# penumbra-zone/decaf377

Hardware: AMD Instinct MI355X
Metric: decaf377 var-base scalar-mults/sec + encodes/sec at 1/2/4/8 MI355X (higher is better)
Workload: dtype u32

## Files before the change

### decaf377_amd/csrc/batch_host.hpp

```cpp
#pragma once
#include <hip/hip_runtime.h>
#include <stdint.h>
#include <stdio.h>
#include <stdlib.h>

#include "dcb.hpp"
#include "straus.hpp"
#include "host_state.hpp"

namespace d377 {

inline int lane_residency(const void* fn, const char* name, int bits, int& lds) {
  if (lds >= 0) return D377_OK;
  int nb = 0;
  HIP_TRY(hipOccupancyMaxActiveBlocksPerMultiprocessor(&nb, fn, BLOCK, 0));
  int pad = 0;
  if (nb > WAVES_PER_SIMD) {
    pad = (160 * 1024) / (WAVES_PER_SIMD + 1) + 1024;
    if (pad > 64 * 1024) HIP_TRY(hipFuncSetAttribute(fn, hipFuncAttributeMaxDynamicSharedMemorySize, pad));
    HIP_TRY(hipOccupancyMaxActiveBlocksPerMultiprocessor(&nb, fn, BLOCK, (size_t)pad));
  }
  if (getenv("D377_DEBUG_RESIDENCY"))
    fprintf(stderr, "d377: %s<%d>: %d workgroups per CU with %d bytes of LDS padding\n", name, bits, nb, pad);
  if (nb < 1 || nb > WAVES_PER_SIMD)
    return fail(D377_ERR_INIT, "residency of %s does not match the lane sets of the scratch areas", name);
  lds = pad;
  return D377_OK;
}

inline int straus_scratch_reserve(DeviceState& d, hipStream_t s, size_t terms, const char* in_capture, const char* no_memory,
                                  uint32_t** tab, uint32_t** dig) {
  const size_t tab_words = d.resident_lanes() * terms * VB_ENTRIES * BM_ENTRY_WORDS;
  const size_t need = (tab_words + d.resident_lanes() * BM_WINDOWS) * sizeof(uint32_t);
  if (need > d.bm_cap) {
    if (ScratchGuard::capturing(s)) return fail(D377_ERR_ARG, "%s", in_capture);
    int rc;
    if ((rc = d.vb_guard.drain())) return rc;
    if (d.bm_scratch) HIP_TRY(hipFree(d.bm_scratch));
    d.bm_scratch = nullptr; d.bm_cap = 0;
    if (hipMalloc(&d.bm_scratch, need) != hipSuccess) {
      (void)hipGetLastError();
      return fail(D377_ERR_HIP, "%s", no_memory);
    }
    d.bm_cap = need;
  }
  *tab = d.bm_scratch;
  *dig = d.bm_scratch + tab_words;
  return D377_OK;
}

inline DcbScratch lane_chunks(const DeviceState& d, size_t count, int* grid, int kmax = DCB_K) {
  const size_t places = (size_t)d.cus * WAVES_PER_SIMD;
  const ChunkDeal c = deal_chunks((count + BLOCK - 1) / BLOCK, places, (size_t)kmax, (size_t)d.cus * 64);
  DcbScratch dcb{d.dcb_scratch, d.slot_pool, d.cus * WAVES_PER_SIMD, (int)c.per_lane, d.dcb_sets * BLOCK, (int)c.extra, d.pool_health};
  dcb.prio = c.nchunks <= 2 * places ? 1 : 0;
  *grid = (int)c.nchunks;
  return dcb;
}

template <class Body>
int device_slice(DeviceState& d, Body&& body) {
  HIP_TRY(hipSetDevice(d.id));
  int rc = D377_OK;
  SyncOnError guard{&rc, d.id, d.stream, nullptr};
  rc = [&]() -> int {
    StarveCheck starve{d, d.stream};
    int r;
    if ((r = starve.before())) return r;
    if ((r = body())) return r;
    if ((r = starve.after())) return r;
    HIP_TRY(hipStreamSynchronize(d.stream));
    return starve.verdict();
  }();
  return rc;
}

inline int sums_out_reserve(DeviceState& d, size_t n, bool want_xyzt, uint64_t** xyzt_dev) {
  int rc;
  if ((rc = ensure(d, 2, n * (want_xyzt ? 32 + 128 : 32)))) return rc;
  *xyzt_dev = want_xyzt ? reinterpret_cast<uint64_t*>(d.buf[2] + n * 32) : nullptr;
  return D377_OK;
}
inline int sums_out_copy(DeviceState& d, size_t n, uint8_t* out32, uint64_t* xyzt_out) {
  HIP_TRY(hipMemcpyAsync(out32, d.buf[2], n * 32, hipMemcpyDeviceToHost, d.stream));
  if (xyzt_out) HIP_TRY(hipMemcpyAsync(xyzt_out, d.buf[2] + n * 32, n * 128, hipMemcpyDeviceToHost, d.stream));
// ... 5 lines not shown
```

### decaf377_amd/csrc/batch_msm.hip

```cpp
#include <hip/hip_runtime.h>
#include <stdint.h>
#include <stdlib.h>
#include <string.h>

#include "../../include/decaf377_amd.h"
#include "curve.hpp"
#include "device_util.hpp"
#include "dcb.hpp"
#include "quad_ops.hpp"
#include "row_ops.hpp"
#include "straus.hpp"
#include "straus_tab.hpp"
#include "host_state.hpp"
#include "batch_host.hpp"

using namespace d377;

namespace {

constexpr int BM_MAX = D377_BATCH_MSM_MAX_TERMS;
static_assert(BM_MAX == 8, "a window's digits of the m points of a sum are the eight nibbles of one word");
static_assert(VB_ENTRIES == 9, "straus_sum stores entries 0 .. 8 of every point's table");

template <bool ENCODED>
__global__ void __launch_bounds__(BLOCK, WAVES_PER_SIMD)
k_batch_msm_lane(SqrtTables T, const void* pts_in, const uint8_t* scalar32, int m, size_t n, uint8_t* out32, uint64_t* xyzt_out,
                 uint8_t* status, uint32_t* tab, uint32_t* dig, DcbScratch dcb) {
  __shared__ uint32_t lds_pow_[ENCODED ? POW_TAB * NL * BLOCK : 1];
  LdsPowTab pt;
  pt.col = lds_pow_ + (ENCODED ? threadIdx.x : 0);
  D377_DCB_BEGIN(out32);
  StrausTab st{tab, dig, (size_t)dcb.nslots * BLOCK, io.lane};
  dcb_rounds<0, true>(n, io, pt,
    [&](size_t, int) {},
    [&](size_t i, int j, const uint32_t (*)[8], bool) {
      const size_t first = i * (size_t)m;
      const ge r = straus_sum(st, m, [&](int p, uint32_t k[8]) { load32(scalar32, first + (size_t)p, k); }, [&](int p, ge* g) -> bool {
        if (ENCODED) {
          uint32_t w[8];
          load32(reinterpret_cast<const uint8_t*>(pts_in), first + (size_t)p, w);
          const uint32_t bad = ge_decompress(T, pt, w, g);
          status[first + (size_t)p] = (uint8_t)bad;
          return bad != 0;
        }
        *g = load_ge_mont256(reinterpret_cast<const uint64_t*>(pts_in), first + (size_t)p);
        D377_INVARIANT(T, *g, !fe_is_zero(g->z));
        return fe_is_zero(g->z);
      }, DCB_WANT_T);
      if (xyzt_out) store_ge_mont256(xyzt_out, i, ge_double_fast(r, true));
      dcb_put(io, j, ge_dcb_from_half(r, false));
    });
  D377_DCB_END();
}

struct OneIO {
  uint32_t st[4][8], parked_[8], out[8];
  __device__ __forceinline__ void put(int s, int, const uint32_t* w) { for (int k = 0; k < 8; ++k) st[s][k] = w[k]; }
  __device__ __forceinline__ void get(int s, int, uint32_t* w) const { for (int k = 0; k < 8; ++k) w[k] = st[s][k]; }
  __device__ __forceinline__ void park(int, const uint32_t* w) { for (int k = 0; k < 8; ++k) parked_[k] = w[k]; }
  __device__ __forceinline__ void parked(int, uint32_t* w) const { for (int k = 0; k < 8; ++k) w[k] = parked_[k]; }
  __device__ __forceinline__ void emit(int, const uint32_t* w) { for (int k = 0; k < 8; ++k) out[k] = w[k]; }
};
using row::RQ_WORDS;
template <bool ENCODED>
__global__ void __launch_bounds__(64)
k_batch_msm_wave(SqrtTables T, const void* pts_in, const uint8_t* scalar32, int m, size_t n, uint8_t* out32, uint64_t* xyzt_out,
                 uint8_t* status) {
  extern __shared__ uint32_t tab[];
  __shared__ uint32_t xrec[2 * RQ_WORDS];
  __shared__ uint32_t sdg[BM_MAX][8];
  const int t = threadIdx.x;
  (void)n;
  const ge r = straus_wave_sum<ENCODED>(T, pts_in, scalar32, (size_t)blockIdx.x * (size_t)m, m, status, tab, xrec, sdg);
  if (xyzt_out && t == 0) store_ge_mont256(xyzt_out, blockIdx.x, ge_double_fast(r, true));
  OneIO io;
  dcb_put(io, 0, ge_dcb_from_half(r, false));
  dcb_finish_with(io, 1, [](const fe& c) { return row::fe_invert_wave(c); });
  if (t == 0) store32(out32, blockIdx.x, io.out);
}

int batch_msm_launch(DeviceState& d, hipStream_t s, bool encoded, const void* pts_in, const uint8_t* scalars, size_t m, size_t n,
                     uint8_t* out32, uint64_t* xyzt_out, uint8_t* status) {
  if (n == 0) return D377_OK;
  const SqrtTables T = d.tables();
  const size_t wave_max = 4 * (size_t)d.tuned(D377_TUNE_TINY_MAX, (long long)d.cus * 4);
  if (n <= wave_max) {
    const size_t lds = m * row::RQ_TAB_ENTRIES * RQ_WORDS * sizeof(uint32_t);
    if (encoded) hipLaunchKernelGGL(k_batch_msm_wave<true>, dim3((unsigned)n), dim3(64), lds, s, T, pts_in, scalars, (int)m, n, out32, xyzt_out, status);
    else hipLaunchKernelGGL(k_batch_msm_wave<false>, dim3((unsigned)n), dim3(64), lds, s, T, pts_in, scalars, (int)m, n, out32, xyzt_out, status);
    HIP_TRY(hipGetLastError());
    return D377_OK;
  }
  const void* fn = encoded ? reinterpret_cast<const void*>(k_batch_msm_lane<true>) : reinterpret_cast<const void*>(k_batch_msm_lane<false>);
  int& lds = d.bm_lds[encoded ? 1 : 0];
  int rc;
  if ((rc = lane_residency(fn, "k_batch_msm_lane", encoded, lds))) return rc;
  GuardScope vb{d.vb_guard, s};
  uint32_t *tab, *dig;
  if ((rc = straus_scratch_reserve(d, s, m,
         "batch_msm_small: the table scratch must grow, which cannot happen inside a stream capture -- run one call with this many terms first",
         "batch_msm_small: hipMalloc of the table scratch failed (0.23 GB per term on 256 CUs)", &tab, &dig))) return rc;
  if ((rc = vb.acquire())) return rc;
  int grid;
  const DcbScratch dcb = lane_chunks(d, n, &grid);
  if (encoded)
    hipLaunchKernelGGL(k_batch_msm_lane<true>, dim3((unsigned)grid), dim3(BLOCK), lds, s, T, pts_in, scalars, (int)m, n, out32, xyzt_out, status, tab, dig, dcb);
  else
    hipLaunchKernelGGL(k_batch_msm_lane<false>, dim3((unsigned)grid), dim3(BLOCK), lds, s, T, pts_in, scalars, (int)m, n, out32, xyzt_out, status, tab, dig, dcb);
  HIP_TRY(hipGetLastError());
  return vb.finish();
}

int check_terms(size_t m) {
  if (m < 1 || m > (size_t)BM_MAX) return fail(D377_ERR_ARG, "%s", "batch_msm_small: 1 .. 8 terms per sum (D377_BATCH_MSM_MAX_TERMS); d377_msm for one long sum");
  return D377_OK;
}

int batch_msm_one(DeviceState& d, bool encoded, const uint8_t* pts_in, const uint8_t* scalars, size_t m, size_t n, uint8_t* out32,
                  uint64_t* xyzt_out, uint8_t* status) {
  if (n == 0) return D377_OK;
  return device_slice(d, [&]() -> int {
    const size_t rec = encoded ? 32 : 128, terms = n * m;
    int r;
    uint64_t* xyzt_dev;
    if ((r = ensure(d, 0, terms * rec))) return r;
    if ((r = ensure(d, 1, terms * 32))) return r;
    if ((r = sums_out_reserve(d, n, xyzt_out != nullptr, &xyzt_dev))) return r;
    if (encoded && (r = ensure(d, 3, terms))) return r;
    HIP_TRY(hipMemcpyAsync(d.buf[0], pts_in, terms * rec, hipMemcpyHostToDevice, d.stream));
    HIP_TRY(hipMemcpyAsync(d.buf[1], scalars, terms * 32, hipMemcpyHostToDevice, d.stream));
    if ((r = batch_msm_launch(d, d.stream, encoded, d.buf[0], d.buf[1], m, n, d.buf[2], xyzt_dev, d.buf[3]))) return r;
    if ((r = sums_out_copy(d, n, out32, xyzt_out))) return r;
    if (encoded) HIP_TRY(hipMemcpyAsync(status, d.buf[3], terms, hipMemcpyDeviceToHost, d.stream));
    return D377_OK;
  });
}

int batch_msm_host(d377_ctx* ctx, bool encoded, const void* pts_in, const uint8_t* scalars, size_t m, size_t n, uint8_t* out32,
                   uint64_t* xyzt_out, uint8_t* status) {
  if (!ctx) return fail(D377_ERR_ARG, "%s", "null context");
  int rc = check_terms(m);
  if (rc) return rc;
  if (n && (!pts_in || !scalars || !out32 || (encoded && !status))) return fail(D377_ERR_ARG, "%s", "null buffer");
  if (n == 0) return D377_OK;
  std::lock_guard<std::mutex> lock(ctx->mu);
  const size_t rec = encoded ? 32 : 128;
  return slice_over_devices(ctx, n, [&](size_t k, size_t lo, size_t cnt) {
    return batch_msm_one(ctx->devs[k], encoded, (const uint8_t*)pts_in + lo * m * rec, scalars + lo * m * 32, m, cnt, out32 + lo * 32,
                         xyzt_out ? xyzt_out + lo * 16 : nullptr, encoded ? status + lo * m : nullptr);
  });
}

int batch_msm_dev(d377_ctx* ctx, int dev, void* stream, bool encoded, const void* pts_in, const uint8_t* scalars, size_t m, size_t n,
                  uint8_t* out32, uint64_t* xyzt_out, uint8_t* status) {
  if (!ctx) return fail(D377_ERR_ARG, "%s", "null context");
  if (dev < 0 || (size_t)dev >= ctx->devs.size()) return fail(D377_ERR_ARG, "%s", "device index out of range");
  int rc = check_terms(m);
  if (rc) return rc;
  if (n && (!pts_in || !scalars || !out32 || (encoded && !status))) return fail(D377_ERR_ARG, "%s", "null buffer");
  if (!aligned16(pts_in) || !aligned16(scalars) || !aligned16(out32) || !aligned16(xyzt_out))
    return fail(D377_ERR_ARG, "%s", "device record buffers must be 16-byte aligned");
// ... 29 lines not shown
```

### decaf377_amd/csrc/batch_msm_long.hip

```cpp
#include <hip/hip_runtime.h>
#include <stdint.h>
#include <stdio.h>
#include <stdlib.h>
#include <string.h>

#include "../../include/decaf377_amd.h"
#include "curve.hpp"
#include "device_util.hpp"
#include "dcb.hpp"
#include "quad_ops.hpp"
#include "row_ops.hpp"
#include "straus.hpp"
#include "straus_tab.hpp"
#include "host_state.hpp"
#include "batch_host.hpp"
#include "codec_chunked.hpp"
#include "batch_msm_long_plan.hpp"
#include "msm_long_fold.hpp"

using namespace d377;

namespace {

constexpr size_t BML_MAX = D377_BATCH_MSM_LONG_MAX_TERMS;
static_assert(BML_GROUP_MAX == D377_BATCH_MSM_MAX_TERMS, "a group is one chain of the small sums");
static_assert(VB_ENTRIES == 9, "straus_sum stores entries 0 .. 8 of every point's table");

template <bool ENCODED>
__global__ void __launch_bounds__(BLOCK, WAVES_PER_SIMD)
k_msm_long_lane(SqrtTables T, const void* pts_in, const uint8_t* scalar32, LongPlan plan, size_t np, uint64_t* partials,
                uint8_t* status, uint32_t* tab, uint32_t* dig, DcbScratch dcb) {
  __shared__ uint32_t lds_pow_[ENCODED ? POW_TAB * NL * BLOCK : 1];
  LdsPowTab pt;
  pt.col = lds_pow_ + (ENCODED ? threadIdx.x : 0);
  D377_DCB_BEGIN(partials);
  StrausTab st{tab, dig, (size_t)dcb.nslots * BLOCK, io.lane};
  dcb_rounds<0, false>(np, io, pt,
    [&](size_t, int) {},
    [&](size_t i, int, const uint32_t (*)[8], bool) {
      const size_t s = i / plan.g, q = i % plan.g;
      const size_t first = s * plan.m + plan.first(q);
      const int live = (int)plan.count(q);
      const ge r = straus_sum(st, (int)plan.b, [&](int p, uint32_t k[8]) {
        if (p < live) { load32(scalar32, first + (size_t)p, k); return; }
#pragma unroll
        for (int w = 0; w < 8; ++w) k[w] = 0;
      }, [&](int p, ge* g) -> bool {
        if (p >= live) { *g = ge_identity(); return true; }
        if (ENCODED) {
          uint32_t w[8];
          load32(reinterpret_cast<const uint8_t*>(pts_in), first + (size_t)p, w);
          const uint32_t bad = ge_decompress(T, pt, w, g);
          status[first + (size_t)p] = (uint8_t)bad;
          return bad != 0;
        }
        *g = load_ge_mont256(reinterpret_cast<const uint64_t*>(pts_in), first + (size_t)p);
        D377_INVARIANT(T, *g, !fe_is_zero(g->z));
        return fe_is_zero(g->z);
      }, DCB_WANT_T);
      store_ge_mont256(partials, i, ge_double_fast(r, true));
    });
  D377_DCB_END();
}

using row::RQ_WORDS;
template <bool ENCODED>
__global__ void __launch_bounds__(64)
k_msm_long_wave(SqrtTables T, const void* pts_in, const uint8_t* scalar32, LongPlan plan, size_t np, uint64_t* partials,
                uint8_t* status) {
  extern __shared__ uint32_t tab[];
  __shared__ uint32_t xrec[2 * RQ_WORDS];
  __shared__ uint32_t sdg[BML_GROUP_MAX][8];
  const size_t part = blockIdx.x;
  if (part >= np) return;
  const size_t gq = part % plan.g;
  const ge r = straus_wave_sum<ENCODED>(T, pts_in, scalar32, (part / plan.g) * plan.m + plan.first(gq), (int)plan.count(gq), status,
                                        tab, xrec, sdg);
  if (threadIdx.x == 0) store_ge_mont256(partials, part, ge_double_fast(r, true));
}

__global__ void __launch_bounds__(BLOCK) k_msm_long_fold(const uint64_t* in, size_t c, size_t nsums, uint64_t* out) {
  const size_t oc = fold_out(c), total = nsums * oc;
  for (size_t L = (size_t)blockIdx.x * BLOCK + threadIdx.x; L < total; L += (size_t)gridDim.x * BLOCK) {
    const size_t s = L / oc, f = L % oc;
    const size_t lo = s * c + f * BML_FOLD;
    const int cnt = (int)fold_count(c, f);
    uint32_t acc[32];
    load_record128(in, lo, acc);
#pragma unroll 1
    for (int j = 1; j < cnt; ++j) {
      uint32_t q[32], r[32];
      load_record128(in, lo + (size_t)j, q);
      ge_add_raw_words(acc, q, false, r);
#pragma unroll
      for (int w = 0; w < 32; ++w) acc[w] = r[w];
    }
    store_record128(out, L, acc);
  }
}

int fail_size(int code, const char* fmt, size_t a) {
  char msg[256];
  snprintf(msg, sizeof msg, fmt, a);
  return fail(code, "%s", msg);
}
// ... 33 lines not shown
  uint64_t* partials = reinterpret_cast<uint64_t*>(d.bml_partials);
  const size_t np = n * g;
  uint64_t* half[2] = {partials + np * 16, partials + (np + n * fold_out(g)) * 16};

  const uint64_t* cur = partials;
  int turn = 0;
  for (size_t c = g; c > 1; c = fold_out(c)) {
    const size_t oc = fold_out(c), lanes = n * oc;
    uint64_t* dst = (oc == 1 && xyzt_out) ? xyzt_out : half[turn];
    size_t grid = (lanes + BLOCK - 1) / BLOCK;
    if (grid > (size_t)d.cus * 8) grid = (size_t)d.cus * 8;
    hipLaunchKernelGGL(k_msm_long_fold, dim3((unsigned)grid), dim3(BLOCK), 0, s, cur, c, n, dst);
    HIP_TRY(hipGetLastError());
    cur = dst;
    turn ^= 1;
  }

  int grid;
  const DcbScratch dcb = lane_chunks(d, n, &grid);
  return codec_chunked_launch(d, s, false, cur, n, out32, nullptr, grid, dcb);
}

}

namespace {

int batch_msm_long_launch(DeviceState& d, hipStream_t s, bool encoded, const void* pts_in, const uint8_t* scalars, size_t m, size_t n,
                          uint8_t* out32, uint64_t* xyzt_out, uint8_t* status) {
  if (n == 0) return D377_OK;
  const SqrtTables T = d.tables();
  const LongPlan plan = long_plan(m);
  const size_t np = n * plan.g;
  if (!codec_chunked_ok(d))
    return fail(D377_ERR_INIT, "residency of %s does not match the lane sets of the scratch areas", "k_compress_chunked");
  GuardScope vb{d.vb_guard, s};
  int rc;
  uint64_t* partials = nullptr;
  if ((rc = long_sums_partials(d, s, n, plan.g, &partials))) return rc;

  const size_t wave_max = 4 * (size_t)d.tuned(D377_TUNE_TINY_MAX, (long long)d.cus * 4);
  if (np <= wave_max) {
    if ((rc = vb.acquire())) return rc;
    const size_t lds = plan.b * row::RQ_TAB_ENTRIES * RQ_WORDS * sizeof(uint32_t);
    if (encoded) hipLaunchKernelGGL(k_msm_long_wave<true>, dim3((unsigned)np), dim3(64), lds, s, T, pts_in, scalars, plan, np, partials, status);
    else hipLaunchKernelGGL(k_msm_long_wave<false>, dim3((unsigned)np), dim3(64), lds, s, T, pts_in, scalars, plan, np, partials, status);
    HIP_TRY(hipGetLastError());
  } else {
    const void* fn = encoded ? reinterpret_cast<const void*>(k_msm_long_lane<true>) : reinterpret_cast<const void*>(k_msm_long_lane<false>);
    int& lds = d.bml_lds[encoded ? 1 : 0];
    if ((rc = lane_residency(fn, "k_msm_long_lane", encoded, lds))) return rc;
    uint32_t *tab, *dig;
    if ((rc = straus_scratch_reserve(d, s, plan.b,
           "batch_msm_long: the table scratch must grow, which cannot happen inside a stream capture",
           "batch_msm_long: hipMalloc of the table scratch failed (0.23 GB per term of a group on 256 CUs)", &tab, &dig))) return rc;
    if ((rc = vb.acquire())) return rc;
    int grid;
    const DcbScratch dcb = lane_chunks(d, np, &grid);
    if (encoded)
      hipLaunchKernelGGL(k_msm_long_lane<true>, dim3((unsigned)grid), dim3(BLOCK), lds, s, T, pts_in, scalars, plan, np, partials, status, tab, dig, dcb);
    else
      hipLaunchKernelGGL(k_msm_long_lane<false>, dim3((unsigned)grid), dim3(BLOCK), lds, s, T, pts_in, scalars, plan, np, partials, status, tab, dig, dcb);
    HIP_TRY(hipGetLastError());
  }

  if ((rc = long_sums_fold_compress(d, s, n, plan.g, out32, xyzt_out))) return rc;
  return vb.finish();
}

int batch_msm_long_one(DeviceState& d, bool encoded, const uint8_t* pts_in, const uint8_t* scalars, size_t m, size_t n, uint8_t* out32,
                       uint64_t* xyzt_out, uint8_t* status) {
  if (n == 0) return D377_OK;
  return device_slice(d, [&]() -> int {
    const size_t rec = encoded ? 32 : 128, terms = n * m;
    int r;
    uint64_t* xyzt_dev;
    if ((r = ensure(d, 0, terms * rec))) return r;
    if ((r = ensure(d, 1, terms * 32))) return r;
    if ((r = sums_out_reserve(d, n, xyzt_out != nullptr, &xyzt_dev))) return r;
    if (encoded && (r = ensure(d, 3, terms))) return r;
    HIP_TRY(hipMemcpyAsync(d.buf[0], pts_in, terms * rec, hipMemcpyHostToDevice, d.stream));
    HIP_TRY(hipMemcpyAsync(d.buf[1], scalars, terms * 32, hipMemcpyHostToDevice, d.stream));
    if ((r = batch_msm_long_launch(d, d.stream, encoded, d.buf[0], d.buf[1], m, n, d.buf[2], xyzt_dev, d.buf[3]))) return r;
    if ((r = sums_out_copy(d, n, out32, xyzt_out))) return r;
    if (encoded) HIP_TRY(hipMemcpyAsync(status, d.buf[3], terms, hipMemcpyDeviceToHost, d.stream));
    return D377_OK;
  });
}

int batch_msm_long_host(d377_ctx* ctx, bool encoded, const void* pts_in, const uint8_t* scalars, size_t m, size_t n, uint8_t* out32,
                        uint64_t* xyzt_out, uint8_t* status) {
  if (m < 1 || m > BML_MAX)
    return fail_size(D377_ERR_ARG, "batch_msm_long: m = %zu: 1 .. 4096 terms per sum (D377_BATCH_MSM_LONG_MAX_TERMS); d377_msm for longer sums", m);
  if (n) {
    if (!pts_in) return fail(D377_ERR_ARG, "batch_msm_long: null buffer: %s", encoded ? "enc32" : "xyzt");
    if (!scalars) return fail(D377_ERR_ARG, "batch_msm_long: null buffer: %s", "scalar32");
    if (!out32) return fail(D377_ERR_ARG, "batch_msm_long: null buffer: %s", "enc32_out");
    if (encoded && !status) return fail(D377_ERR_ARG, "batch_msm_long: null buffer: %s", "status");
  }
  if (!ctx) return fail(D377_ERR_ARG, "%s", "batch_msm_long: null context (ctx)");
  if (n == 0) return D377_OK;
  if (m <= BML_GROUP_MAX)
    return encoded ? d377_batch_msm_small_encoded(ctx, (const uint8_t*)pts_in, scalars, m, n, out32, xyzt_out, status)
                   : d377_batch_msm_small(ctx, (const uint64_t*)pts_in, scalars, m, n, out32, xyzt_out);
  std::lock_guard<std::mutex> lock(ctx->mu);
  const size_t rec = encoded ? 32 : 128;
  return slice_over_devices(ctx, n, [&](size_t k, size_t lo, size_t cnt) {
    return batch_msm_long_one(ctx->devs[k], encoded, (const uint8_t*)pts_in + lo * m * rec, scalars + lo * m * 32, m, cnt, out32 + lo * 32,
                              xyzt_out ? xyzt_out + lo * 16 : nullptr, encoded ? status + lo * m : nullptr);
  });
}

}

extern "C" {
// ... 12 lines not shown
```

### decaf377_amd/csrc/batch_msm_mixed.hip

```cpp
#include <hip/hip_runtime.h>
#include <stdint.h>
#include <stdio.h>
#include <stdlib.h>
#include <string.h>
#include <mutex>

#include "../../include/decaf377_amd.h"
#include "curve.hpp"
#include "device_util.hpp"
#include "dcb.hpp"
#include "straus.hpp"
#include "straus_tab.hpp"
#include "comb_tabs.hpp"
#include "mixed_sum.hpp"
#include "host_state.hpp"
#include "batch_host.hpp"

using namespace d377;

namespace {

constexpr int MX_VAR_MAX = D377_BATCH_MSM_MIXED_MAX_VAR;
constexpr int MX_FIXED_MAX = D377_FIXED_BASES_MAX;
static_assert(MX_VAR_MAX == D377_BATCH_MSM_MAX_TERMS && MX_VAR_MAX == 8, "a window's digits of the v points of a sum are the eight nibbles of one word");
static_assert(VB_ENTRIES == 9, "straus_sum stores entries 0 .. 8 of every point's table");

template <int BITS, bool ENCODED>
__global__ void __launch_bounds__(BLOCK, WAVES_PER_SIMD)
k_batch_msm_mixed_lane(SqrtTables T, const uint32_t* tabs, const int* base_index, const uint8_t* fixed_scalar32, int m, int t,
                       const void* pts_in, const uint8_t* var_scalar32, int v, size_t n, uint8_t* out32, uint64_t* xyzt_out,
                       uint8_t* status, uint32_t* tab, uint32_t* dig, DcbScratch dcb) {
  __shared__ uint32_t lds_pow_[ENCODED ? POW_TAB * NL * BLOCK : 1];
  LdsPowTab pt;
  pt.col = lds_pow_ + (ENCODED ? threadIdx.x : 0);
  D377_DCB_BEGIN(out32);
  StrausTab st{tab, dig, (size_t)dcb.nslots * BLOCK, io.lane};
  const CombTabs<BITS> ft{tabs};
  dcb_rounds<0, true>(n, io, pt,
    [&](size_t, int) {},
    [&](size_t i, int j, const uint32_t (*)[8], bool) {
      const size_t vfirst = i * (size_t)v, ffirst = i * (size_t)t;
      const ge r = mixed_half_sum<BITS>(st, v,
        [&](int p, uint32_t k[8]) { load32(var_scalar32, vfirst + (size_t)p, k); },
        [&](int p, ge* g) -> bool {
          if (ENCODED) {
            uint32_t w[8];
            load32(reinterpret_cast<const uint8_t*>(pts_in), vfirst + (size_t)p, w);
            const uint32_t bad = ge_decompress(T, pt, w, g);
            status[vfirst + (size_t)p] = (uint8_t)bad;
            return bad != 0;
          }
          *g = load_ge_mont256(reinterpret_cast<const uint64_t*>(pts_in), vfirst + (size_t)p);
          D377_INVARIANT(T, *g, !fe_is_zero(g->z));
          return fe_is_zero(g->z);
        },
        t, [&](int p, uint32_t k[8]) -> int {
          const int b = base_index[ffirst + (size_t)p];
          load32(fixed_scalar32, ffirst + (size_t)p, k);
          fr_reduce_words(k);
          fr_half_words(k);
          const uint32_t keep = (uint32_t)b < (uint32_t)m ? ~0u : 0u;
#pragma unroll
          for (int q = 0; q < 8; ++q) k[q] &= keep;
          return (int)((uint32_t)b & keep);
        }, ft);
      D377_INVARIANT(T, r, true);
      if (xyzt_out) store_ge_mont256(xyzt_out, i, ge_double_fast(r, true));
      dcb_put(io, j, ge_dcb_from_half(r, false));
    });
  D377_DCB_END();
}

struct MixedArgs {
  const uint32_t* combs;
  int m, bits;
  const int* index;
  const uint8_t* fixed_scalars;
  size_t t;
  bool encoded;
  const void* pts_in;
  const uint8_t* var_scalars;
  size_t v;
};

int mixed_launch(DeviceState& d, hipStream_t s, const MixedArgs& a, size_t n, uint8_t* out32, uint64_t* xyzt_out, uint8_t* status) {
  if (n == 0) return D377_OK;
  const SqrtTables T = d.tables();
  return with_width(a.bits, "batch_msm_mixed: the registration's comb width is none of 8, 12, 16, 18", [&](auto bb) -> int {
    constexpr int BITS = decltype(bb)::value;
    const void* fn = a.encoded ? reinterpret_cast<const void*>(k_batch_msm_mixed_lane<BITS, true>)
                               : reinterpret_cast<const void*>(k_batch_msm_mixed_lane<BITS, false>);
    int& lds = d.bmx_lds[a.encoded ? 1 : 0][width_slot(BITS)];
    int rc;
    if ((rc = lane_residency(fn, "k_batch_msm_mixed_lane", BITS, lds))) return rc;
    GuardScope vb{d.vb_guard, s};
    uint32_t *tab, *dig;
    if ((rc = straus_scratch_reserve(d, s, a.v,
           "batch_msm_mixed: the table scratch must grow, which cannot happen inside a stream capture",
           "batch_msm_mixed: hipMalloc of the table scratch failed (0.23 GB per variable term on 256 CUs)", &tab, &dig))) return rc;
    if ((rc = vb.acquire())) return rc;
    int grid;
    const DcbScratch dcb = lane_chunks(d, n, &grid);
    if (a.encoded)
      hipLaunchKernelGGL((k_batch_msm_mixed_lane<BITS, true>), dim3((unsigned)grid), dim3(BLOCK), lds, s, T, a.combs, a.index,
                         a.fixed_scalars, a.m, (int)a.t, a.pts_in, a.var_scalars, (int)a.v, n, out32, xyzt_out, status, tab, dig, dcb);
    else
      hipLaunchKernelGGL((k_batch_msm_mixed_lane<BITS, false>), dim3((unsigned)grid), dim3(BLOCK), lds, s, T, a.combs, a.index,
                         a.fixed_scalars, a.m, (int)a.t, a.pts_in, a.var_scalars, (int)a.v, n, out32, xyzt_out, status, tab, dig, dcb);
    HIP_TRY(hipGetLastError());
    return vb.finish();
  });
}

int mixed_one(DeviceState& d, const FixedBases& fb, const uint32_t* combs, const int* index, const uint8_t* fixed_scalars, size_t t,
              bool encoded, const uint8_t* pts_in, const uint8_t* var_scalars, size_t v, size_t n, uint8_t* out32,
              uint64_t* xyzt_out, uint8_t* status) {
  if (n == 0) return D377_OK;
  return device_slice(d, [&]() -> int {
    const size_t rec = encoded ? 32 : 128, vterms = n * v, fterms = n * t;
    const size_t idx_off = fterms * 32, var_off = idx_off + ((fterms * sizeof(int) + 15) & ~(size_t)15);
    int r;
    uint64_t* xyzt_dev;
    if ((r = ensure(d, 0, vterms * rec))) return r;
    if ((r = ensure(d, 1, var_off + vterms * 32))) return r;
    if ((r = sums_out_reserve(d, n, xyzt_out != nullptr, &xyzt_dev))) return r;
    if (encoded && (r = ensure(d, 3, vterms))) return r;
    HIP_TRY(hipMemcpyAsync(d.buf[0], pts_in, vterms * rec, hipMemcpyHostToDevice, d.stream));
    HIP_TRY(hipMemcpyAsync(d.buf[1], fixed_scalars, fterms * 32, hipMemcpyHostToDevice, d.stream));
    HIP_TRY(hipMemcpyAsync(d.buf[1] + idx_off, index, fterms * sizeof(int), hipMemcpyHostToDevice, d.stream));
    HIP_TRY(hipMemcpyAsync(d.buf[1] + var_off, var_scalars, vterms * 32, hipMemcpyHostToDevice, d.stream));
    const MixedArgs a{combs, (int)fb.m, fb.bits, reinterpret_cast<const int*>(d.buf[1] + idx_off), d.buf[1], t, encoded, d.buf[0],
                      d.buf[1] + var_off, v};
    if ((r = mixed_launch(d, d.stream, a, n, d.buf[2], xyzt_dev, d.buf[3]))) return r;
    if ((r = sums_out_copy(d, n, out32, xyzt_out))) return r;
    if (encoded) HIP_TRY(hipMemcpyAsync(status, d.buf[3], vterms, hipMemcpyDeviceToHost, d.stream));
    return D377_OK;
  });
}

int mixed_host(const char* who, d377_ctx* ctx, int64_t handle, const int* base_index, const uint8_t* fixed_scalar32, size_t t,
               bool encoded, const void* pts_in, const uint8_t* var_scalar32, size_t v, size_t n, uint8_t* enc32_out,
               uint64_t* xyzt_out, uint8_t* status) {
  if (v < 1 || v > (size_t)MX_VAR_MAX)
    return fail(D377_ERR_ARG, "%s: v must be 1 .. 8 variable terms per sum (D377_BATCH_MSM_MIXED_MAX_VAR); d377_batch_fixed_msm_indexed serves v = 0", who);
  if (t < 1 || t > (size_t)MX_FIXED_MAX)
    return fail(D377_ERR_ARG, "%s: t must be 1 .. 64 fixed terms per sum (D377_FIXED_BASES_MAX); d377_batch_msm_small serves t = 0", who);
  if (n) {
    const char* null_arg = !base_index ? "base_index" : !fixed_scalar32 ? "fixed_scalar32" : !pts_in ? (encoded ? "enc32" : "xyzt")
                         : !var_scalar32 ? "var_scalar32" : !enc32_out ? "enc32_out" : (encoded && !status) ? "status" : nullptr;
    if (null_arg) {
      snprintf(d377_g_err, sizeof d377_g_err, "%s: %s is null", who, null_arg);
      return D377_ERR_ARG;
    }
  }
  if (!ctx) return fail(D377_ERR_ARG, "%s: ctx is null", who);
  std::lock_guard<std::mutex> lock(ctx->mu);
  const FixedBases* fb = fixed_bases_find(ctx, handle);
  if (!fb) return fail(D377_ERR_ARG, "%s: handle is not a live registration of this context", who);
  if (n > SIZE_MAX / 128 / (t > v ? t : v)) return fail(D377_ERR_ARG, "%s: n x t or n x v overflows", who);
  const size_t fterms = n * t;
  const int m = (int)fb->m;
// ... 38 lines not shown
```

### decaf377_amd/csrc/mixed_sum.hpp

```cpp
#pragma once
#include <stdint.h>

#include "curve.hpp"
#include "straus.hpp"

namespace d377 {

template <int BITS, class Tab, class LoadScalar, class LoadPoint, class TLoad, class FTab>
D377_HD ge mixed_half_sum(Tab& st, int v, LoadScalar load_var_scalar, LoadPoint load_point, int t, TLoad&& tload, const FTab& ftab) {
  const ge hv = straus_sum(st, v, load_var_scalar, load_point, true);
  const ge hf = ge_fixed_msm_indexed_w8<BITS>(t, tload, ftab, true);
  return ge_add(hv, hf);
}

}
```

### decaf377_amd/csrc/straus.hpp

```cpp
#pragma once
#include <stdint.h>

#include "curve.hpp"

namespace d377 {

constexpr int BM_WINDOWS = 64;

D377_HD int nibble_digit(uint32_t word, int p) { return (int)(((word >> (4 * p)) & 15u) ^ 8u) - 8; }

template <class Reload>
D377_HD ge ge_add_cached_reload(const ge& p, gec& q, bool neg, bool with_t, Reload reload) {
  fe a = fe_mul(fe_sub_nc(p.y, p.x), q.ymx);
  fe b = fe_mul(fe_add(p.y, p.x), q.ypx);
  fe c = fe_mul(p.t, q.kt);
  fe d = fe_mul(p.z, q.z2);
#if defined(__HIPCC__)
  asm volatile("" ::: "memory");
#endif
  reload(q);
#if defined(__HIPCC__)
  asm volatile("" ::: "memory");
#endif
  fe e = fe_sub(b, a), h = fe_add(b, a);
  fe dmc = fe_sub(d, c), dpc = fe_add(d, c);
  fe f = fe_select(neg, dpc, dmc), g = fe_select(neg, dmc, dpc);
  ge r;
  r.x = fe_mul(e, f); r.y = fe_mul(g, h); r.z = fe_mul(f, g);
  r.t = p.t;
  if (with_t) r.t = fe_mul(e, h);
  return r;
}

template <class Tab, class LoadScalar, class LoadPoint>
D377_HD ge straus_sum(Tab& st, int m, LoadScalar load_scalar, LoadPoint load_point, bool want_t = false) {
  uint32_t deadmask = 0;
#pragma unroll 1
  for (int p = 0; p < m; ++p) {
    ge g;
    if (load_point(p, &g)) deadmask |= 1u << p;
    gec id;
    id.ypx = fe_const(FE_ONE); id.ymx = fe_const(FE_ONE); id.z2 = fe_dbl(fe_const(FE_ONE)); id.kt = fe_zero();
    st.store(p, 0, id);
    const gec pc = ge_to_cached(g);
    st.store(p, 1, pc);
    ge acc = ge_double_fast(g, true);
    st.store(p, 2, ge_to_cached(acc));
#pragma unroll 1
    for (int j = 3; j <= 8; ++j) {
      acc = ge_add_cached(acc, pc, false, true);
      st.store(p, j, ge_to_cached(acc));
    }
  }
  {
    uint32_t W[BM_WINDOWS];
#pragma unroll
    for (int w = 0; w < BM_WINDOWS; ++w) W[w] = 0;
#pragma unroll 1
    for (int p = 0; p < m; ++p) {
      uint32_t k[8], dg[8];
      load_scalar(p, k);
      fr_reduce_words(k);
      fr_half_words(k);
      fr_recode_signed16(k, dg);
      const uint32_t live = ((deadmask >> p) & 1u) ? 0u : 15u;
#pragma unroll
      for (int wi = 0; wi < 8; ++wi)
#pragma unroll
        for (int b = 0; b < 8; ++b) W[8 * wi + b] |= ((dg[wi] >> (4 * b)) & live) << (4 * p);
    }
#pragma unroll
    for (int w = 0; w < BM_WINDOWS; ++w) st.dig_store(w, W[w]);
  }
  ge r = ge_identity();
  uint32_t wn = st.dig_load(BM_WINDOWS - 1);
  int d = nibble_digit(wn, 0);
  bool neg = d < 0;
  gec e = st.load(0, neg ? -d : d, neg);
#pragma unroll 1
  for (int i = BM_WINDOWS - 1; i >= 0; --i) {
    const uint32_t wc = wn;
    wn = st.dig_load(i > 0 ? i - 1 : 0);
    if (i != BM_WINDOWS - 1) {
#pragma unroll 1
      for (int j = 0; j < 4; ++j) r = ge_double_neg(r, j == 3);
    }
#pragma unroll 1
    for (int p = 0; p < m; ++p) {
      const bool neg_cur = neg;
      const bool more = p + 1 < m;
      const int np = more ? p + 1 : 0;
      d = nibble_digit(more ? wc : wn, np);
      neg = d < 0;
      const int nj = neg ? -d : d;
      r = ge_add_cached_reload(r, e, neg_cur, more || (i == 0 && want_t), [&](gec& q) { q = st.load(np, nj, neg); });
    }
  }
  return r;
}

}
```

### decaf377_amd/csrc/straus_tab.hpp

```cpp
#pragma once
#include <hip/hip_runtime.h>
#include <stdint.h>

#include "curve.hpp"
#include "device_util.hpp"
#include "quad_ops.hpp"
#include "row_ops.hpp"
#include "straus.hpp"

namespace d377 {

struct StrausTab {
  uint32_t* tab;
  uint32_t* dig;
  size_t nthreads, tid;
  __device__ __forceinline__ uint32_t* entry(int p, int j) const { return tab + (((size_t)p * VB_ENTRIES + j) * nthreads + tid) * BM_ENTRY_WORDS; }
  __device__ __forceinline__ void store(int p, int j, const gec& c) {
    uint32_t* q = entry(p, j);
    slot_store(q, c.ypx); slot_store(q + SLOT, c.ymx); slot_store(q + 2 * SLOT, c.z2); slot_store(q + 3 * SLOT, c.kt);
  }
  __device__ __forceinline__ gec load(int p, int j, bool swap) const {
    const uint32_t* q = entry(p, j);
    gec c;
    c.ypx = slot_load(q + (swap ? SLOT : 0));
    c.ymx = slot_load(q + (swap ? 0 : SLOT));
    c.z2 = slot_load(q + 2 * SLOT);
    c.kt = slot_load(q + 3 * SLOT);
    return c;
  }
  __device__ __forceinline__ void dig_store(int w, uint32_t v) { dig[(size_t)w * nthreads + tid] = v; }
  __device__ __forceinline__ uint32_t dig_load(int w) const { return dig[(size_t)w * nthreads + tid]; }
};

static_assert(POW_TAB * 64 <= row::RQ_TAB_ENTRIES * row::RQ_WORDS, "row_sqrt_powers' scratch must fit in one point's LDS table");

template <bool ENCODED>
__device__ __forceinline__ ge straus_wave_sum(const SqrtTables& T, const void* pts_in, const uint8_t* scalar32, size_t first, int m,
                                              uint8_t* status, uint32_t* tab, uint32_t* xrec, uint32_t (*sdg)[8]) {
  using row::RQ_WORDS;
  const int t = threadIdx.x;
  const row::RowK K = row::row_consts();
  const row::RowSel S = row::row_sel();
#pragma unroll 1
  for (int base = 0; base < m; base += 4) {
    const int pj = t & 3;
    const bool mine = base + pj < m;
    const size_t e_mine = first + (size_t)(mine ? base + pj : 0);
    ge g;
    bool skip = !mine;
    if (ENCODED) {
      uint32_t w[8];
      load32(reinterpret_cast<const uint8_t*>(pts_in), e_mine, w);
      if (t < 4) row::row_store_from_fe(xrec + 16 * t, ge_decompress_den(w));
      __syncthreads();
      const row::RowPowers pw = row::row_sqrt_powers(xrec[t], tab + base * row::RQ_TAB_ENTRIES * RQ_WORDS, t, K);
      __syncthreads();
      xrec[t] = pw.v; xrec[RQ_WORDS + t] = pw.uv;
      __syncthreads();
      const fe pv = row::row_load_to_fe(xrec + 16 * pj), puv = row::row_load_to_fe(xrec + RQ_WORDS + 16 * pj);
      __syncthreads();
      const uint32_t bad = ge_decompress_from_powers(T, w, pv, puv, &g);
      if (t < 4 && mine) status[e_mine] = (uint8_t)bad;
      skip |= bad != 0;
    } else {
      g = load_ge_mont256(reinterpret_cast<const uint64_t*>(pts_in), e_mine);
      skip |= fe_is_zero(g.z);
      D377_INVARIANT(T, g, t < 4 && !skip);
    }
#pragma unroll 1
    for (int j = 0; j < 4 && base + j < m; ++j) {
      uint32_t k[8], dg[8];
      load32(scalar32, first + (size_t)(base + j), k);
      fr_reduce_words(k);
      fr_half_words(k);
      fr_recode_signed16(k, dg);
      if (pj == j && t < 16) row::row_store_from_fe(xrec + 16 * (t >> 2), fe_pick(t >> 2, g.x, g.y, g.z, g.t));
      __syncthreads();
      const bool dead = __shfl((int)skip, j) != 0;
      if (t < 8) sdg[base + j][t] = dead ? 0u : dg[t];
      row::rq_build_table(dead ? row::rq_identity(S) : xrec[t], tab + (base + j) * row::RQ_TAB_ENTRIES * RQ_WORDS, S, K);
// ... 24 lines not shown
```

Before: 75.43 million.

## Use lean Straus chain with packed table entries and shared identity record

Replaces straus_sum with straus_sum_lean in the lane kernels of batch_msm, batch_msm_long and batch_msm_mixed. The table now stores entries 1..8 in a packed slot format with a narrower field type (fes), and entry 0 is served from one shared identity record. The chain also starts at the top window without a redundant doubling. This cuts the per-lane global scratch footprint and the load/store traffic of the table in the memory-bound chain. In exchange it adds pack/unpack work, a new field representation and a dependency on a device-side identity buffer.

```diff
diff --git a/decaf377_amd/csrc/batch_host.hpp b/decaf377_amd/csrc/batch_host.hpp
--- a/decaf377_amd/csrc/batch_host.hpp
+++ b/decaf377_amd/csrc/batch_host.hpp
@@ -30,7 +30,7 @@
 
 inline int straus_scratch_reserve(DeviceState& d, hipStream_t s, size_t terms, const char* in_capture, const char* no_memory,
                                   uint32_t** tab, uint32_t** dig) {
-  const size_t tab_words = d.resident_lanes() * terms * VB_ENTRIES * BM_ENTRY_WORDS;
+  const size_t tab_words = d.resident_lanes() * terms * (VB_ENTRIES - 1) * VB_ENTRY_WORDS;
   const size_t need = (tab_words + d.resident_lanes() * BM_WINDOWS) * sizeof(uint32_t);
   if (need > d.bm_cap) {
     if (ScratchGuard::capturing(s)) return fail(D377_ERR_ARG, "%s", in_capture);
diff --git a/decaf377_amd/csrc/batch_msm.hip b/decaf377_amd/csrc/batch_msm.hip
--- a/decaf377_amd/csrc/batch_msm.hip
+++ b/decaf377_amd/csrc/batch_msm.hip
@@ -20,26 +20,26 @@
 
 constexpr int BM_MAX = D377_BATCH_MSM_MAX_TERMS;
 static_assert(BM_MAX == 8, "a window's digits of the m points of a sum are the eight nibbles of one word");
-static_assert(VB_ENTRIES == 9, "straus_sum stores entries 0 .. 8 of every point's table");
+static_assert(StrausTab::STORED == 8, "straus_sum_lean stores entries 1 .. 8 of every point's table; entry 0 is the shared identity record");
 
 template <bool ENCODED>
 __global__ void __launch_bounds__(BLOCK, WAVES_PER_SIMD)
 k_batch_msm_lane(SqrtTables T, const void* pts_in, const uint8_t* scalar32, int m, size_t n, uint8_t* out32, uint64_t* xyzt_out,
-                 uint8_t* status, uint32_t* tab, uint32_t* dig, DcbScratch dcb) {
+                 uint8_t* status, uint32_t* tab, uint32_t* dig, const uint32_t* vb_identity, DcbScratch dcb) {
   __shared__ uint32_t lds_pow_[ENCODED ? POW_TAB * NL * BLOCK : 1];
   LdsPowTab pt;
   pt.col = lds_pow_ + (ENCODED ? threadIdx.x : 0);
   D377_DCB_BEGIN(out32);
-  StrausTab st{tab, dig, (size_t)dcb.nslots * BLOCK, io.lane};
+  StrausTab st{tab, dig, vb_identity, (size_t)dcb.nslots * BLOCK, io.lane};
   dcb_rounds<0, true>(n, io, pt,
     [&](size_t, int) {},
     [&](size_t i, int j, const uint32_t (*)[8], bool) {
       const size_t first = i * (size_t)m;
-      const ge r = straus_sum(st, m, [&](int p, uint32_t k[8]) { load32(scalar32, first + (size_t)p, k); }, [&](int p, ge* g) -> bool {
+      const ge r = straus_sum_lean(st, m, [&](int p, uint32_t k[8]) { load32(scalar32, first + (size_t)p, k); }, [&](int p, ge* g) -> bool {
         if (ENCODED) {
           uint32_t w[8];
           load32(reinterpret_cast<const uint8_t*>(pts_in), first + (size_t)p, w);
-          const uint32_t bad = ge_decompress(T, pt, w, g);
+          const uint32_t bad = ge_decompress<fes>(T, pt, w, g);
           status[first + (size_t)p] = (uint8_t)bad;
           return bad != 0;
         }
@@ -99,14 +99,14 @@
   uint32_t *tab, *dig;
   if ((rc = straus_scratch_reserve(d, s, m,
          "batch_msm_small: the table scratch must grow, which cannot happen inside a stream capture -- run one call with this many terms first",
-         "batch_msm_small: hipMalloc of the table scratch failed (0.23 GB per term on 256 CUs)", &tab, &dig))) return rc;
+         "batch_msm_small: hipMalloc of the table scratch failed (0.13 GB per term on 256 CUs)", &tab, &dig))) return rc;
   if ((rc = vb.acquire())) return rc;
   int grid;
   const DcbScratch dcb = lane_chunks(d, n, &grid);
   if (encoded)
-    hipLaunchKernelGGL(k_batch_msm_lane<true>, dim3((unsigned)grid), dim3(BLOCK), lds, s, T, pts_in, scalars, (int)m, n, out32, xyzt_out, status, tab, dig, dcb);
+    hipLaunchKernelGGL(k_batch_msm_lane<true>, dim3((unsigned)grid), dim3(BLOCK), lds, s, T, pts_in, scalars, (int)m, n, out32, xyzt_out, status, tab, dig, (const uint32_t*)d.vb_identity, dcb);
   else
-    hipLaunchKernelGGL(k_batch_msm_lane<false>, dim3((unsigned)grid), dim3(BLOCK), lds, s, T, pts_in, scalars, (int)m, n, out32, xyzt_out, status, tab, dig, dcb);
+    hipLaunchKernelGGL(k_batch_msm_lane<false>, dim3((unsigned)grid), dim3(BLOCK), lds, s, T, pts_in, scalars, (int)m, n, out32, xyzt_out, status, tab, dig, (const uint32_t*)d.vb_identity, dcb);
   HIP_TRY(hipGetLastError());
   return vb.finish();
 }
diff --git a/decaf377_amd/csrc/batch_msm_long.hip b/decaf377_amd/csrc/batch_msm_long.hip
--- a/decaf377_amd/csrc/batch_msm_long.hip
+++ b/decaf377_amd/csrc/batch_msm_long.hip
@@ -24,24 +24,24 @@
 
 constexpr size_t BML_MAX = D377_BATCH_MSM_LONG_MAX_TERMS;
 static_assert(BML_GROUP_MAX == D377_BATCH_MSM_MAX_TERMS, "a group is one chain of the small sums");
-static_assert(VB_ENTRIES == 9, "straus_sum stores entries 0 .. 8 of every point's table");
+static_assert(StrausTab::STORED == 8, "straus_sum_lean stores entries 1 .. 8 of every point's table; entry 0 is the shared identity record");
 
 template <bool ENCODED>
 __global__ void __launch_bounds__(BLOCK, WAVES_PER_SIMD)
 k_msm_long_lane(SqrtTables T, const void* pts_in, const uint8_t* scalar32, LongPlan plan, size_t np, uint64_t* partials,
-                uint8_t* status, uint32_t* tab, uint32_t* dig, DcbScratch dcb) {
+                uint8_t* status, uint32_t* tab, uint32_t* dig, const uint32_t* vb_identity, DcbScratch dcb) {
   __shared__ uint32_t lds_pow_[ENCODED ? POW_TAB * NL * BLOCK : 1];
   LdsPowTab pt;
   pt.col = lds_pow_ + (ENCODED ? threadIdx.x : 0);
   D377_DCB_BEGIN(partials);
-  StrausTab st{tab, dig, (size_t)dcb.nslots * BLOCK, io.lane};
+  StrausTab st{tab, dig, vb_identity, (size_t)dcb.nslots * BLOCK, io.lane};
   dcb_rounds<0, false>(np, io, pt,
     [&](size_t, int) {},
     [&](size_t i, int, const uint32_t (*)[8], bool) {
       const size_t s = i / plan.g, q = i % plan.g;
       const size_t first = s * plan.m + plan.first(q);
       const int live = (int)plan.count(q);
-      const ge r = straus_sum(st, (int)plan.b, [&](int p, uint32_t k[8]) {
+      const ge r = straus_sum_lean(st, (int)plan.b, [&](int p, uint32_t k[8]) {
         if (p < live) { load32(scalar32, first + (size_t)p, k); return; }
 #pragma unroll
         for (int w = 0; w < 8; ++w) k[w] = 0;
@@ -50,7 +50,7 @@
         if (ENCODED) {
           uint32_t w[8];
           load32(reinterpret_cast<const uint8_t*>(pts_in), first + (size_t)p, w);
-          const uint32_t bad = ge_decompress(T, pt, w, g);
+          const uint32_t bad = ge_decompress<fes>(T, pt, w, g);
           status[first + (size_t)p] = (uint8_t)bad;
           return bad != 0;
         }
@@ -190,14 +190,14 @@
     uint32_t *tab, *dig;
     if ((rc = straus_scratch_reserve(d, s, plan.b,
            "batch_msm_long: the table scratch must grow, which cannot happen inside a stream capture",
-           "batch_msm_long: hipMalloc of the table scratch failed (0.23 GB per term of a group on 256 CUs)", &tab, &dig))) return rc;
+           "batch_msm_long: hipMalloc of the table scratch failed (0.13 GB per term of a group on 256 CUs)", &tab, &dig))) return rc;
     if ((rc = vb.acquire())) return rc;
     int grid;
     const DcbScratch dcb = lane_chunks(d, np, &grid);
     if (encoded)
-      hipLaunchKernelGGL(k_msm_long_lane<true>, dim3((unsigned)grid), dim3(BLOCK), lds, s, T, pts_in, scalars, plan, np, partials, status, tab, dig, dcb);
+      hipLaunchKernelGGL(k_msm_long_lane<true>, dim3((unsigned)grid), dim3(BLOCK), lds, s, T, pts_in, scalars, plan, np, partials, status, tab, dig, (const uint32_t*)d.vb_identity, dcb);
     else
-      hipLaunchKernelGGL(k_msm_long_lane<false>, dim3((unsigned)grid), dim3(BLOCK), lds, s, T, pts_in, scalars, plan, np, partials, status, tab, dig, dcb);
+      hipLaunchKernelGGL(k_msm_long_lane<false>, dim3((unsigned)grid), dim3(BLOCK), lds, s, T, pts_in, scalars, plan, np, partials, status, tab, dig, (const uint32_t*)d.vb_identity, dcb);
     HIP_TRY(hipGetLastError());
   }
 
diff --git a/decaf377_amd/csrc/batch_msm_mixed.hip b/decaf377_amd/csrc/batch_msm_mixed.hip
--- a/decaf377_amd/csrc/batch_msm_mixed.hip
+++ b/decaf377_amd/csrc/batch_msm_mixed.hip
@@ -23,18 +23,18 @@
 constexpr int MX_VAR_MAX = D377_BATCH_MSM_MIXED_MAX_VAR;
 constexpr int MX_FIXED_MAX = D377_FIXED_BASES_MAX;
 static_assert(MX_VAR_MAX == D377_BATCH_MSM_MAX_TERMS && MX_VAR_MAX == 8, "a window's digits of the v points of a sum are the eight nibbles of one word");
-static_assert(VB_ENTRIES == 9, "straus_sum stores entries 0 .. 8 of every point's table");
+static_assert(StrausTab::STORED == 8, "straus_sum_lean stores entries 1 .. 8 of every point's table; entry 0 is the shared identity record");
 
 template <int BITS, bool ENCODED>
 __global__ void __launch_bounds__(BLOCK, WAVES_PER_SIMD)
 k_batch_msm_mixed_lane(SqrtTables T, const uint32_t* tabs, const int* base_index, const uint8_t* fixed_scalar32, int m, int t,
                        const void* pts_in, const uint8_t* var_scalar32, int v, size_t n, uint8_t* out32, uint64_t* xyzt_out,
-                       uint8_t* status, uint32_t* tab, uint32_t* dig, DcbScratch dcb) {
+                       uint8_t* status, uint32_t* tab, uint32_t* dig, const uint32_t* vb_identity, DcbScratch dcb) {
   __shared__ uint32_t lds_pow_[ENCODED ? POW_TAB * NL * BLOCK : 1];
   LdsPowTab pt;
   pt.col = lds_pow_ + (ENCODED ? threadIdx.x : 0);
   D377_DCB_BEGIN(out32);
-  StrausTab st{tab, dig, (size_t)dcb.nslots * BLOCK, io.lane};
+  StrausTab st{tab, dig, vb_identity, (size_t)dcb.nslots * BLOCK, io.lane};
   const CombTabs<BITS> ft{tabs};
   dcb_rounds<0, true>(n, io, pt,
     [&](size_t, int) {},
@@ -46,7 +46,7 @@
           if (ENCODED) {
             uint32_t w[8];
             load32(reinterpret_cast<const uint8_t*>(pts_in), vfirst + (size_t)p, w);
-            const uint32_t bad = ge_decompress(T, pt, w, g);
+            const uint32_t bad = ge_decompress<fes>(T, pt, w, g);
             status[vfirst + (size_t)p] = (uint8_t)bad;
             return bad != 0;
           }
@@ -97,16 +97,18 @@
     uint32_t *tab, *dig;
     if ((rc = straus_scratch_reserve(d, s, a.v,
            "batch_msm_mixed: the table scratch must grow, which cannot happen inside a stream capture",
-           "batch_msm_mixed: hipMalloc of the table scratch failed (0.23 GB per variable term on 256 CUs)", &tab, &dig))) return rc;
+           "batch_msm_mixed: hipMalloc of the table scratch failed (0.13 GB per variable term on 256 CUs)", &tab, &dig))) return rc;
     if ((rc = vb.acquire())) return rc;
     int grid;
     const DcbScratch dcb = lane_chunks(d, n, &grid);
     if (a.encoded)
       hipLaunchKernelGGL((k_batch_msm_mixed_lane<BITS, true>), dim3((unsigned)grid), dim3(BLOCK), lds, s, T, a.combs, a.index,
-                         a.fixed_scalars, a.m, (int)a.t, a.pts_in, a.var_scalars, (int)a.v, n, out32, xyzt_out, status, tab, dig, dcb);
+                         a.fixed_scalars, a.m, (int)a.t, a.pts_in, a.var_scalars, (int)a.v, n, out32, xyzt_out, status, tab, dig,
+                         (const uint32_t*)d.vb_identity, dcb);
     else
       hipLaunchKernelGGL((k_batch_msm_mixed_lane<BITS, false>), dim3((unsigned)grid), dim3(BLOCK), lds, s, T, a.combs, a.index,
-                         a.fixed_scalars, a.m, (int)a.t, a.pts_in, a.var_scalars, (int)a.v, n, out32, xyzt_out, status, tab, dig, dcb);
+                         a.fixed_scalars, a.m, (int)a.t, a.pts_in, a.var_scalars, (int)a.v, n, out32, xyzt_out, status, tab, dig,
+                         (const uint32_t*)d.vb_identity, dcb);
     HIP_TRY(hipGetLastError());
     return vb.finish();
   });
diff --git a/decaf377_amd/csrc/mixed_sum.hpp b/decaf377_amd/csrc/mixed_sum.hpp
--- a/decaf377_amd/csrc/mixed_sum.hpp
+++ b/decaf377_amd/csrc/mixed_sum.hpp
@@ -8,7 +8,9 @@
 
 template <int BITS, class Tab, class LoadScalar, class LoadPoint, class TLoad, class FTab>
 D377_HD ge mixed_half_sum(Tab& st, int v, LoadScalar load_var_scalar, LoadPoint load_point, int t, TLoad&& tload, const FTab& ftab) {
-  const ge hv = straus_sum(st, v, load_var_scalar, load_point, true);
+  ge hv;
+  if constexpr (tab_shares_identity<Tab>::value) hv = straus_sum_lean(st, v, load_var_scalar, load_point, true);
+  else hv = straus_sum(st, v, load_var_scalar, load_point, true);
   const ge hf = ge_fixed_msm_indexed_w8<BITS>(t, tload, ftab, true);
   return ge_add(hv, hf);
 }
diff --git a/decaf377_amd/csrc/straus.hpp b/decaf377_amd/csrc/straus.hpp
--- a/decaf377_amd/csrc/straus.hpp
+++ b/decaf377_amd/csrc/straus.hpp
@@ -9,12 +9,12 @@
 
 D377_HD int nibble_digit(uint32_t word, int p) { return (int)(((word >> (4 * p)) & 15u) ^ 8u) - 8; }
 
-template <class Reload>
-D377_HD ge ge_add_cached_reload(const ge& p, gec& q, bool neg, bool with_t, Reload reload) {
-  fe a = fe_mul(fe_sub_nc(p.y, p.x), q.ymx);
-  fe b = fe_mul(fe_add(p.y, p.x), q.ypx);
-  fe c = fe_mul(p.t, q.kt);
-  fe d = fe_mul(p.z, q.z2);
+template <class F, class Reload>
+D377_HD ge_of<F> ge_add_cached_reload(const ge_of<F>& p, gec_of<F>& q, bool neg, bool with_t, Reload reload) {
+  F a = fe_mul(fe_sub_nc(p.y, p.x), q.ymx);
+  F b = fe_mul(fe_add(p.y, p.x), q.ypx);
+  F c = fe_mul(p.t, q.kt);
+  F d = fe_mul(p.z, q.z2);
 #if defined(__HIPCC__)
   asm volatile("" ::: "memory");
 #endif
@@ -22,10 +22,10 @@
 #if defined(__HIPCC__)
   asm volatile("" ::: "memory");
 #endif
-  fe e = fe_sub(b, a), h = fe_add(b, a);
-  fe dmc = fe_sub(d, c), dpc = fe_add(d, c);
-  fe f = fe_select(neg, dpc, dmc), g = fe_select(neg, dmc, dpc);
-  ge r;
+  F e = fe_sub(b, a), h = fe_add(b, a);
+  F dmc = fe_sub(d, c), dpc = fe_add(d, c);
+  F f = fe_select(neg, dpc, dmc), g = fe_select(neg, dmc, dpc);
+  ge_of<F> r;
   r.x = fe_mul(e, f); r.y = fe_mul(g, h); r.z = fe_mul(f, g);
   r.t = p.t;
   if (with_t) r.t = fe_mul(e, h);
@@ -99,4 +99,82 @@
   return r;
 }
 
+constexpr int BM_TOP_WINDOW = BM_WINDOWS - 2;
+template <class Tab, class LoadScalar, class LoadPoint>
+D377_HD ge straus_sum_lean(Tab& st, int m, LoadScalar load_scalar, LoadPoint load_point, bool want_t = false) {
+  static_assert(tab_shares_identity<Tab>::value, "straus_sum_lean never stores entry 0: the table serves load(p, 0, .) from a shared identity record");
+  using F = fes;
+  uint32_t deadmask = 0;
+#pragma unroll 1
+  for (int p = 0; p < m; ++p) {
+    ge g0;
+    if (load_point(p, &g0)) deadmask |= 1u << p;
+    const ge_of<F> g = ge_as<F>(g0);
+    const gec_of<F> pc = ge_to_cached(g);
+    st.store(p, 1, pc);
+    ge_of<F> acc = ge_double_fast(g, true);
+    st.store(p, 2, ge_to_cached(acc));
+#pragma unroll 1
+    for (int j = 3; j <= 8; ++j) {
+      acc = ge_add_cached(acc, pc, false, true);
+      st.store(p, j, ge_to_cached(acc));
+    }
+  }
+  {
+    uint32_t W[BM_WINDOWS];
+#pragma unroll
+    for (int w = 0; w < BM_WINDOWS; ++w) W[w] = 0;
+#if defined(__clang__)
+#pragma clang loop unroll(disable) vectorize(disable) interleave(disable)
+#endif
+    for (int p = 0; p < m; ++p) {
+      uint32_t k[8], dg[8];
+      load_scalar(p, k);
+      fr_reduce_words(k);
+      fr_half_words(k);
+      fr_recode_signed16(k, dg);
+      const uint32_t live = ((deadmask >> p) & 1u) ? 0u : 15u;
+      D377_B(bound_require(live == 0 || (fr_digit(dg, 63) == 0 && fr_digit(dg, 62) >= 0 && fr_digit(dg, 62) <= 5),
+                           "lean Straus chain: the scalar is not below r"));
+#pragma unroll
+      for (int wi = 0; wi < 8; ++wi)
+#pragma unroll
+        for (int b = 0; b < 8; ++b) W[8 * wi + b] |= ((dg[wi] >> (4 * b)) & live) << (4 * p);
+    }
+#pragma unroll
+    for (int w = 0; w <= BM_TOP_WINDOW; ++w) st.dig_store(w, W[w]);
+  }
+  uint32_t wc = st.dig_load(BM_TOP_WINDOW), wn = st.dig_load(BM_TOP_WINDOW - 1);
+  ge_of<F> r;
+  {
+    const gec_of<F> s = st.load(0, nibble_digit(wc, 0) & 7, false);
+    r.x = fe_carry(fe_sub(s.ypx, s.ymx)); r.y = fe_carry(fe_add(s.ypx, s.ymx)); r.z = fe_carry(s.z2);
+    r.t = fe_as<F>(fe_zero());
+    if (m > 1) r.t = fe_mul(s.kt, fe_as<F>(fe_const(FE_2_OVER_K)));
+  }
+  int d = m > 1 ? nibble_digit(wc, 1) : nibble_digit(wn, 0);
+  bool neg = d < 0;
+  gec_of<F> e = st.load(m > 1 ? 1 : 0, neg ? -d : d, neg);
+#pragma unroll 1
+  for (int i = BM_TOP_WINDOW; i >= 0; --i) {
+    if (i != BM_TOP_WINDOW) {
+      wc = wn;
+      wn = st.dig_load(i > 0 ? i - 1 : 0);
+#pragma unroll 1
+      for (int j = 0; j < 4; ++j) r = ge_double_neg_sq(r, j == 3);
+    }
+#pragma unroll 1
+    for (int p = i == BM_TOP_WINDOW ? 1 : 0; p < m; ++p) {
+      const bool neg_cur = neg;
+      const bool more = p + 1 < m;
+      const int np = more ? p + 1 : 0;
+      d = nibble_digit(more ? wc : wn, np);
+      neg = d < 0;
+      const int nj = neg ? -d : d;
+      r = ge_add_cached_reload(r, e, neg_cur, more || (i == 0 && want_t), [&](gec_of<F>& q) { q = st.load(np, nj, neg); });
+    }
+  }
+  return ge_unsigned(r);
 }
+
+}
diff --git a/decaf377_amd/csrc/straus_tab.hpp b/decaf377_amd/csrc/straus_tab.hpp
--- a/decaf377_amd/csrc/straus_tab.hpp
+++ b/decaf377_amd/csrc/straus_tab.hpp
@@ -11,21 +11,25 @@
 namespace d377 {
 
 struct StrausTab {
+  static constexpr bool shared_identity = true;
+  static constexpr int STORED = VB_ENTRIES - 1;
   uint32_t* tab;
   uint32_t* dig;
+  const uint32_t* ident;
   size_t nthreads, tid;
-  __device__ __forceinline__ uint32_t* entry(int p, int j) const { return tab + (((size_t)p * VB_ENTRIES + j) * nthreads + tid) * BM_ENTRY_WORDS; }
-  __device__ __forceinline__ void store(int p, int j, const gec& c) {
+  __device__ __forceinline__ uint32_t* entry(int p, int j) const { return tab + (((size_t)p * STORED + (size_t)(j - 1)) * nthreads + tid) * VB_ENTRY_WORDS; }
+  __device__ __forceinline__ void store(int p, int j, const gec_of<fes>& c) {
     uint32_t* q = entry(p, j);
-    slot_store(q, c.ypx); slot_store(q + SLOT, c.ymx); slot_store(q + 2 * SLOT, c.z2); slot_store(q + 3 * SLOT, c.kt);
+    slot_pack_store(q, c.ypx); slot_pack_store(q + PACKED_SLOT, c.ymx);
+    slot_pack_store(q + 2 * PACKED_SLOT, c.z2); slot_pack_store(q + 3 * PACKED_SLOT, c.kt);
   }
-  __device__ __forceinline__ gec load(int p, int j, bool swap) const {
-    const uint32_t* q = entry(p, j);
-    gec c;
-    c.ypx = slot_load(q + (swap ? SLOT : 0));
-    c.ymx = slot_load(q + (swap ? 0 : SLOT));
-    c.z2 = slot_load(q + 2 * SLOT);
-    c.kt = slot_load(q + 3 * SLOT);
+  __device__ __forceinline__ gec_of<fes> load(int p, int j, bool swap) const {
+    const uint32_t* q = j == 0 ? ident : entry(p, j);
+    gec_of<fes> c;
+    c.ypx = slot_unpack_load<fes>(q + (swap ? PACKED_SLOT : 0));
+    c.ymx = slot_unpack_load<fes>(q + (swap ? 0 : PACKED_SLOT));
+    c.z2 = slot_unpack_load<fes>(q + 2 * PACKED_SLOT);
+    c.kt = slot_unpack_load<fes>(q + 3 * PACKED_SLOT);
     return c;
   }
   __device__ __forceinline__ void dig_store(int w, uint32_t v) { dig[(size_t)w * nthreads + tid] = v; }
```

After: 75.40 million, median of 2. Within noise of the previous version (-0.0%).
